# rst-tu-dortmund/teb_local_planner

Measured on AMD Instinct MI355X. Metric: TEB LM iterations/sec (whole node), higher is better.
Workload: dtype f64; 1 GPU; C4: 256 candidate TEBs/GPU x 200 poses at the start (teb_autosize on, the reference default: 193..287 poses, mean 234, after the step), 500 point obstacles (50 dynamic), diff-drive, point footprint, TebConfig defaults, 4 outer x 5 inner; tebs_per_gpu=256, tebs_total=256, poses=200, pose_capacity=288, tebs_ok=256, obstacles=500, jacobian_mode=analytic (closed form), exchange=none (single GPU), binary_hash=10be306ab42698fd, binary_variant_defines=

## Files before the change

### include/teb_amd.h

```cpp
#ifndef TEB_AMD_H_
#define TEB_AMD_H_

#include <stdint.h>

#ifdef __cplusplus
extern "C" {
#endif

#define TEB_AMD_ABI_VERSION 3
#define TEB_AMD_MAX_POSES 944

enum {
  TEB_AMD_OK = 0,
  TEB_AMD_ERR_INVALID_ARG = 1,
  TEB_AMD_ERR_NO_DEVICE = 2,
  TEB_AMD_ERR_HIP = 3,
  TEB_AMD_ERR_CAPACITY = 4,
  TEB_AMD_ERR_UNSUPPORTED = 5
};

enum {
  TEB_AMD_TEB_OK = 0,
  TEB_AMD_TEB_FAILED = 1,
  TEB_AMD_TEB_NONFINITE = 2
// ... 129 lines not shown
typedef struct teb_amd_results {
  int32_t* status;
  int32_t* lm_iterations;
  int32_t* lm_trials;
  double*  chi2;
  double*  cost;
  double*  lambda;
} teb_amd_results_t;

typedef struct teb_amd_handle teb_amd_handle_t;

int  teb_amd_abi_version(void);
const char* teb_amd_last_error(void);
void teb_amd_config_default(teb_amd_config_t* cfg);

enum { TEB_AMD_LAYOUT_AUTO = 0,
       TEB_AMD_LAYOUT_BLOCKS_LDS = 1,
       TEB_AMD_LAYOUT_BAND_LDS = 2,
       TEB_AMD_LAYOUT_BAND_HBM = 3 };
enum { TEB_AMD_HSIG3D_AUTO = 0, TEB_AMD_HSIG3D_WIDE = 1, TEB_AMD_HSIG3D_SMALL = 2 };
typedef struct teb_amd_options {
  int32_t struct_size;
  int32_t layout;
  int32_t fixed_layout;
  int32_t band_ldlt;
  int32_t generic_distance_path;
  int32_t hsig3d_kernel;
  int32_t no_near_cache;
  int32_t multi_cu;
  int32_t multi_cu_timeout_us;
  int32_t speculative_trials;
  int32_t generic_config_path;
  int32_t compile_for_config;
  int32_t reserved[4];
} teb_amd_options_t;
void teb_amd_options_default(teb_amd_options_t* opt);

int  teb_amd_create(const teb_amd_config_t* cfg, int32_t max_tebs, int32_t max_poses,
                    int32_t max_obstacles, int32_t max_obstacle_vertices, int32_t max_via_points,
                    int32_t device, void* stream, teb_amd_handle_t** out);
int  teb_amd_create_ex(const teb_amd_config_t* cfg, int32_t max_tebs, int32_t max_poses,
                       int32_t max_obstacles, int32_t max_obstacle_vertices, int32_t max_via_points,
                       int32_t device, void* stream, const teb_amd_options_t* options, teb_amd_handle_t** out);
void teb_amd_destroy(teb_amd_handle_t* h);
int  teb_amd_set_config(teb_amd_handle_t* h, const teb_amd_config_t* cfg);

int  teb_amd_set_obstacles(teb_amd_handle_t* h, const teb_amd_obstacles_t* obst);
int  teb_amd_set_via_points(teb_amd_handle_t* h, int32_t count, const double* x, const double* y);

int  teb_amd_upload_tebs(teb_amd_handle_t* h, const teb_amd_teb_batch_t* batch);
int  teb_amd_download_tebs(teb_amd_handle_t* h, teb_amd_teb_batch_t* batch);

int  teb_amd_optimize_batch(teb_amd_handle_t* h, int32_t iterations_innerloop, int32_t iterations_outerloop,
                            int32_t compute_cost_afterwards, double obst_cost_scale,
                            double viapoint_cost_scale, int32_t alternative_time_cost);
int  teb_amd_synchronize(teb_amd_handle_t* h);
int  teb_amd_get_results(teb_amd_handle_t* h, teb_amd_results_t* out);

#define TEB_AMD_ITERATION_LOG_ROWS 256
int  teb_amd_set_iteration_log(teb_amd_handle_t* h, int32_t enable);
int  teb_amd_get_iteration_log(teb_amd_handle_t* h, int32_t b, double* rows, int32_t capacity_rows, int32_t* n_rows);

int  teb_amd_select_best(teb_amd_handle_t* h, int32_t last_best, int32_t initial_plan,
                         int32_t* best, double* best_cost);

int  teb_amd_last_launch_info(teb_amd_handle_t* h, int32_t* distance_helpers_per_band, int32_t* solver_helpers_per_band,
                              int32_t* repeated_single_cu);
// ... 106 lines not shown
```

### teb_local_planner_amd/_abi.py

```python
import ctypes as C

import numpy as np

MAX_FOOTPRINT_VERTICES = 64

OK, ERR_INVALID_ARG, ERR_NO_DEVICE, ERR_HIP, ERR_CAPACITY, ERR_UNSUPPORTED = range(6)
MAX_POSES = 944
TEB_OK, TEB_FAILED, TEB_NONFINITE = range(3)
FOOTPRINT_POINT, FOOTPRINT_CIRCULAR, FOOTPRINT_TWO_CIRCLES, FOOTPRINT_LINE, FOOTPRINT_POLYGON = range(5)
OBST_POINT, OBST_CIRCULAR, OBST_LINE, OBST_PILL, OBST_POLYGON = range(5)
ROT_LEFT, ROT_NONE, ROT_RIGHT = range(3)
JACOBIAN_ANALYTIC, JACOBIAN_G2O_NUMERIC = range(2)

c_i32 = C.c_int32
c_f64 = C.c_double
p_i32 = C.POINTER(C.c_int32)
p_f64 = C.POINTER(C.c_double)


class Config(C.Structure):
    _fields_ = [
        ("teb_autosize", c_i32), ("dt_ref", c_f64), ("dt_hysteresis", c_f64),
        ("min_samples", c_i32), ("max_samples", c_i32), ("exact_arc_length", c_i32),
        ("via_points_ordered", c_i32),
# ... 36 lines not shown
        ("count", c_i32), ("type", p_i32), ("ax", p_f64), ("ay", p_f64), ("bx", p_f64), ("by", p_f64),
        ("radius", p_f64), ("vx", p_f64), ("vy", p_f64), ("dynamic", p_i32),
        ("vert_offset", p_i32), ("vert_x", p_f64), ("vert_y", p_f64),
    ]


class TebBatch(C.Structure):
    _fields_ = [
        ("count", c_i32), ("stride", c_i32), ("n", p_i32), ("x", p_f64), ("y", p_f64), ("theta", p_f64),
        ("dt", p_f64), ("has_vel_start", p_i32), ("vel_start", p_f64), ("has_vel_goal", p_i32),
        ("vel_goal", p_f64), ("prefer_rotdir", p_i32), ("via_points_enabled", p_i32),
    ]


class HcpParams(C.Structure):
    _fields_ = [
        ("simple_exploration", c_i32), ("roadmap_graph_no_samples", c_i32), ("roadmap_graph_area_width", c_f64),
        ("roadmap_graph_area_length_scale", c_f64), ("obstacle_heading_threshold", c_f64), ("xy_goal_tolerance", c_f64),
        ("max_number_classes", c_i32), ("max_number_plans_in_current_class", c_i32), ("h_signature_prescaler", c_f64),
        ("h_signature_threshold", c_f64), ("allow_init_with_backwards_motion", c_i32), ("delete_detours_backwards", c_i32),
        ("detours_orientation_tolerance", c_f64), ("length_start_orientation_vector", c_f64),
        ("max_ratio_detours_duration_best_duration", c_f64), ("global_plan_overwrite_orientation", c_i32),
        ("viapoints_all_candidates", c_i32),
    ]


LAYOUT_AUTO, LAYOUT_BLOCKS_LDS, LAYOUT_BAND_LDS, LAYOUT_BAND_HBM = 0, 1, 2, 3
HSIG3D_AUTO, HSIG3D_WIDE, HSIG3D_SMALL = 0, 1, 2


class Options(C.Structure):
    _fields_ = [("struct_size", c_i32), ("layout", c_i32), ("fixed_layout", c_i32), ("band_ldlt", c_i32),
                ("generic_distance_path", c_i32), ("hsig3d_kernel", c_i32), ("no_near_cache", c_i32), ("multi_cu", c_i32),
                ("multi_cu_timeout_us", c_i32), ("speculative_trials", c_i32), ("generic_config_path", c_i32), ("compile_for_config", c_i32), ("reserved", c_i32 * 4)]

    def __init__(self, layout=LAYOUT_AUTO, fixed_layout=False, band_ldlt=False, generic_distance_path=False, hsig3d_kernel=HSIG3D_AUTO,
                 no_near_cache=False, multi_cu=0, multi_cu_timeout_us=0, speculative_trials=0, generic_config_path=False, compile_for_config=0):
        super().__init__()
        self.struct_size = C.sizeof(Options)
        self.layout = {"auto": LAYOUT_AUTO, "cr": LAYOUT_BLOCKS_LDS, "band": LAYOUT_BAND_LDS, "bandg": LAYOUT_BAND_HBM}.get(layout, layout)
        self.fixed_layout = int(fixed_layout)
        self.band_ldlt = int(band_ldlt)
        self.generic_distance_path = int(generic_distance_path)
        self.hsig3d_kernel = {"auto": HSIG3D_AUTO, "wide": HSIG3D_WIDE, "small": HSIG3D_SMALL}.get(hsig3d_kernel, hsig3d_kernel)
        self.no_near_cache = int(no_near_cache)
        self.multi_cu = int(multi_cu)
        self.multi_cu_timeout_us = int(multi_cu_timeout_us)
        self.speculative_trials = int(speculative_trials)
        self.generic_config_path = int(generic_config_path)
        self.compile_for_config = int(compile_for_config)


class Results(C.Structure):
    _fields_ = [
        ("status", p_i32), ("lm_iterations", p_i32), ("lm_trials", p_i32), ("chi2", p_f64),
        ("cost", p_f64), ("lambda_", p_f64),
    ]


def _ptr(a, ty):
    if a is None:
        return C.cast(None, C.POINTER(ty))
    return a.ctypes.data_as(C.POINTER(ty))


def f64(a):
    return np.ascontiguousarray(a, dtype=np.float64)


def i32(a):
    return np.ascontiguousarray(a, dtype=np.int32)


class ObstacleTable:

    def __init__(self):
        self.type, self.ax, self.ay, self.bx, self.by = [], [], [], [], []
        self.radius, self.vx, self.vy, self.dynamic = [], [], [], []
        self.vert_offset, self.vert_x, self.vert_y = [0], [], []
        self._frozen = None

    def _add(self, ty, ax=0.0, ay=0.0, bx=0.0, by=0.0, r=0.0, verts=None, vel=None):
        self._frozen = None
# ... 173 lines not shown
```

### teb_local_planner_amd/csrc/teb_amd.hip

```cpp
#include <hip/hip_runtime.h>

#include <chrono>
#include <cmath>
#include <cstdio>
#include <unistd.h>
#include <cstdlib>
#include <algorithm>
#include <cstring>
#include <limits>
#include <string>
#include <random>
#include <vector>

#include "../../include/teb_amd.h"
#include "../../include/teb_amd_debug.h"
#define TEB_AMD_MAIN_TU
#include "teb_kernel.hpp"
#include "teb_opt_launch.hpp"
#include "teb_fleet.hpp"
#include "teb_strip.hpp"
#include "teb_hsig.hpp"
#include "teb_graph.hpp"
#include "teb_comm.hpp"
#include "teb_rtc.hpp"
// ... 1293 lines not shown
  const size_t w = (size_t)(bt->stride < h->stride ? bt->stride : h->stride) * sizeof(double);
  const size_t hp = (size_t)bt->stride * sizeof(double), dp = (size_t)h->stride * sizeof(double);
  HIPCHK(hipMemcpy2DAsync(bt->x, hp, h->x.p, dp, w, B, hipMemcpyDeviceToHost, h->stream));
  HIPCHK(hipMemcpy2DAsync(bt->y, hp, h->y.p, dp, w, B, hipMemcpyDeviceToHost, h->stream));
  HIPCHK(hipMemcpy2DAsync(bt->theta, hp, h->th.p, dp, w, B, hipMemcpyDeviceToHost, h->stream));
  HIPCHK(hipMemcpy2DAsync(bt->dt, hp, h->dt.p, dp, w, B, hipMemcpyDeviceToHost, h->stream));
  HIPCHK(hipStreamSynchronize(h->stream));
  for (int b = 0; b < B; ++b) bt->n[b] = n[b];
  return TEB_AMD_OK;
}

int teb_amd_optimize_batch(teb_amd_handle_t* h, int32_t inner, int32_t outer, int32_t compute_cost, double obst_cost_scale,
                           double viapoint_cost_scale, int32_t alternative_time_cost) {
  int rc = check_handle(h);
  if (rc) return rc;
  if (inner < 0 || outer < 0) return fail(TEB_AMD_ERR_INVALID_ARG, "negative iteration count");
  const bool fleet = h->fleet.n_scenes > 0;
  if (fleet) {
#ifndef TEB_AMD_HAS_FLEET_UNITS
    return fail(TEB_AMD_ERR_UNSUPPORTED, "fleet launches exist in the product library only; this one is the variant built with [" TEB_AMD_VARIANT_DEFINES "]");
#else
    if (h->cfg.jacobian_mode != TEB_AMD_JACOBIAN_ANALYTIC)
      return fail(TEB_AMD_ERR_INVALID_ARG, "fleet launches need jacobian_mode TEB_AMD_JACOBIAN_ANALYTIC");
    for (int b = 0; b < h->B; ++b)
      if (h->fleet.band_scene[b] >= h->fleet.n_scenes) {
        char buf[160];
        std::snprintf(buf, sizeof buf, "band %d maps to scene %d, but %d scenes are set (teb_amd_set_band_scenes)", b, h->fleet.band_scene[b], h->fleet.n_scenes);
        return fail(TEB_AMD_ERR_INVALID_ARG, buf);
      }
#endif
  }
  OptArgs a;
  std::memset(&a, 0, sizeof a);
  a.inner = inner; a.outer = outer; a.compute_cost = compute_cost; a.no_near_cache = h->opt.no_near_cache != 0; a.band_ldlt = (fleet ? h->fleet.solver : h->solver) == SOLVER_BANDG ? 0 : h->band_ldlt; a.Hband = h->Hband.p; a.hband_stride = h->hband_stride;
  a.obst_scale = obst_cost_scale; a.via_scale = viapoint_cost_scale; a.alt_time = alternative_time_cost;
  if (h->iter_log_on) { a.iter_log = h->iter_log.p; a.iter_log_cap = TEB_AMD_ITERATION_LOG_ROWS; }
  if (h->phase_log_on) a.phase_log = h->phase_log.p;
#ifdef TEB_PROFILE
  a.dbg_H = h->dbg_H.p;
#endif
  h->last_inner = inner;
  return launch(h, a);
}

int teb_amd_set_iteration_log(teb_amd_handle_t* h, int32_t enable) {
  int rc = check_handle(h);
  if (rc) return rc;
  if (enable && !h->iter_log.p) {
    const size_t count = (size_t)h->max_tebs * TEB_AMD_ITERATION_LOG_ROWS * 4;
    HIPCHK(h->iter_log.alloc(count));
    HIPCHK(hipMemsetAsync(h->iter_log.p, 0, count * sizeof(double), h->stream));
  }
  h->iter_log_on = enable != 0;
  return TEB_AMD_OK;
}

static_assert(kPhaseLogSlots == TEB_AMD_PHASE_LOG_SLOTS, "teb_amd_debug.h and teb_device.hpp disagree");
int teb_amd_set_phase_log(teb_amd_handle_t* h, int32_t enable) {
  int rc = check_handle(h);
  if (rc) return rc;
  if (enable && !h->phase_log.p) {
    const size_t count = (size_t)h->max_tebs * kPhaseLogSlots;
    HIPCHK(h->phase_log.alloc(count));
    HIPCHK(hipMemsetAsync(h->phase_log.p, 0, count * sizeof(double), h->stream));
  }
  h->phase_log_on = enable != 0;
  return TEB_AMD_OK;
// ... 1696 lines not shown
```

### teb_local_planner_amd/csrc/teb_device.hpp

```cpp
#pragma once
#include <hip/hip_runtime.h>
#include <stdint.h>

#include "../../include/teb_amd.h"

#define TEB_PF_ALL(X)                                                                                                              \
  X(EXACT_ARC) X(COST_EXPONENT) X(NEW_ASSOCIATION) X(DYNAMIC_EDGES) X(VIA_POINTS) X(NONHOLONOMIC_VELOCITY) X(VELOCITY_EDGES)      \
  X(ACCELERATION_EDGES) X(NONHOLONOMIC_ACCELERATION) X(TIME_OPTIMAL) X(SHORTEST_PATH) X(VELOCITY_OBSTACLE_RATIO) X(RADIUS_FREE)   \
  X(DEBUG_LINEARIZE) X(BAND_LDLT) X(INFLATED) X(NO_NEAR_CACHE) X(DIVERGENCE_DETECTION) X(KIN_DIFF_DRIVE) X(KIN_EDGES)
#define TEB_PF_EXPR_EXACT_ARC (c.exact_arc_length)
#define TEB_PF_DFLT_EXACT_ARC false
#define TEB_PF_EXPR_COST_EXPONENT (c.obstacle_cost_exponent != 1.0 && c.min_obstacle_dist > 0.0)
#define TEB_PF_DFLT_COST_EXPONENT false
#define TEB_PF_EXPR_NEW_ASSOCIATION (!c.legacy_obstacle_association)
#define TEB_PF_DFLT_NEW_ASSOCIATION true
#define TEB_PF_EXPR_DYNAMIC_EDGES (c.include_dynamic_obstacles && c.weight_obstacle != 0)
#define TEB_PF_DFLT_DYNAMIC_EDGES true
#define TEB_PF_HOST_DYNAMIC_EDGES (c.weight_obstacle != 0)
#define TEB_PF_EXPR_VIA_POINTS (sc.nvia > 0 && c.weight_viapoint != 0)
#define TEB_PF_DFLT_VIA_POINTS false
#define TEB_PF_WIDE_VIA_POINTS 1
#define TEB_PF_EXPR_NONHOLONOMIC_VELOCITY (c.max_vel_y == 0)
#define TEB_PF_DFLT_NONHOLONOMIC_VELOCITY true
#define TEB_PF_WIDE_NONHOLONOMIC_VELOCITY 1
// ... 187 lines not shown
  const double* vs;
  const int* has_vg;
  const double* vg;
  const int* rotdir;
  const int* via_en;
  int* status;
  int* optimized;
  int* iters;
  int* last_iters;
  int* trials;
  double* chi2;
  double* cost;
  double* lambda;
  int* assoc_cnt;
  int* assoc;
  int assoc_cap;
  int* assoc_overflow;
  int* legacy_idx;
  int* via_pose;
  int via_cap;
  double* Hbackup;
  size_t hmat_stride;
  long long* clk;
};

struct OptArgs {
  int inner, outer, compute_cost;
  double obst_scale, via_scale;
  int alt_time;
  double* Hband;
  size_t hband_stride;
  int band_ldlt;
  int no_near_cache;
  double* iter_log;
  int iter_log_cap;
  int debug_linearize;
  double debug_weight_multiplier;
  double* dbg_H;
  double* dbg_b;
  double* dbg_chi2;
  double* phase_log;
};
constexpr int kPhaseLogSlots = 9;

}
```

### teb_local_planner_amd/csrc/teb_kernel.hpp

```cpp
#pragma once
#include "teb_edges.hpp"
#include "teb_multicu.hpp"
#include "teb_autoresize_chain.hpp"

namespace tebamd {

#ifdef TEB_PROFILE
#define PROF_DECL long long prof_t0 = 0, prof_wg_t0 = clock64(), prof_acc[8] = {0, 0, 0, 0, 0, 0, 0, 0};
#define PROF_START() prof_t0 = clock64()
#define PROF_END(k) prof_acc[k] += clock64() - prof_t0
#else
#define PROF_DECL const bool plog_ = args.phase_log != nullptr; long long* const plog_acc_ = reinterpret_cast<long long*>(l.red + 40); \
  if (plog_ && threadIdx.x == 0) { for (int q_ = 0; q_ < 9; ++q_) plog_acc_[q_] = 0; plog_acc_[9] = clock64(); }
#define PROF_START() do { if (plog_ && threadIdx.x == 0) plog_acc_[8] = clock64(); } while (0)
#define PROF_END(k) do { if (plog_ && threadIdx.x == 0) plog_acc_[k] += clock64() - plog_acc_[8]; } while (0)
#endif

#ifdef TEB_PROFILE
__device__ long long g_ev_prof[8];
#define EVP_DECL long long evp_t0 = clock64(), evp_t1;
#define EVP(k) do { __builtin_amdgcn_sched_barrier(0); asm volatile("s_waitcnt vmcnt(0) lgkmcnt(0)" ::: "memory"); evp_t1 = clock64(); __builtin_amdgcn_sched_barrier(0); if (blockIdx.x == 0 && threadIdx.x == 1) g_ev_prof[k] += evp_t1 - evp_t0; evp_t0 = evp_t1; } while (0)
__device__ unsigned long long g_assoc_stats[4];
__device__ unsigned long long g_ar_steps[4];
__device__ unsigned long long g_near_recomputed, g_near_queries;
__device__ long long g_lin_prof[16];
#define LNP_DECL long long lnp_t0 = clock64(), lnp_t1;
#define LNP(k) do { __builtin_amdgcn_sched_barrier(0); asm volatile("s_waitcnt vmcnt(0) lgkmcnt(0)" ::: "memory"); lnp_t1 = clock64(); __builtin_amdgcn_sched_barrier(0); if (blockIdx.x == 0 && threadIdx.x == 0) g_lin_prof[k] += lnp_t1 - lnp_t0; lnp_t0 = lnp_t1; } while (0)
#elif defined(TEB_AMD_STAMP)
#define EVP_DECL long long evp_t0 = clock64();
#define EVP(k) do { const long long t_ = clock64(); if ((k) == (TEB_AMD_STAMP) && threadIdx.x == 1) reinterpret_cast<long long*>(l.red + 40)[7] += t_ - evp_t0; evp_t0 = t_; } while (0)
#define LNP_DECL long long lnp_t0 = clock64();
#define LNP(k) do { const long long t_ = clock64(); if ((k) + 10 == (TEB_AMD_STAMP) && threadIdx.x == 0) reinterpret_cast<long long*>(l.red + 40)[7] += t_ - lnp_t0; lnp_t0 = t_; } while (0)
#else
#define EVP_DECL
#define EVP(k)
#define LNP_DECL
#define LNP(k)
#endif
#ifdef TEB_AMD_POINTS_KEEP_GENERIC
#define TEB_IF_FAST(F) if ((F) && sc.fast_points)
#define TEB_IF_NOT_FAST(F) if (!((F) && sc.fast_points))
#else
#define TEB_IF_FAST(F) if constexpr (F)
#define TEB_IF_NOT_FAST(F) if constexpr (!(F))
#endif
enum { SOLVER_BAND = 0, SOLVER_CR = 1, SOLVER_BANDG = 2 };
typedef double teb_v2d __attribute__((ext_vector_type(2)));
constexpr int kBlk = 66;
// ... 538 lines not shown
    const int G = (k0 > 0 || kThreads > 256) ? lanes_per_pose(n - 1 - k0) : 1;
    const int i = k0 + tid / G, sl = tid % G;
    const bool active = i <= n - 2;
    constexpr int EM = JMODE == TEB_AMD_JACOBIAN_G2O_NUMERIC ? 2 : 1;
    const unsigned long long near = active ? dyn_near_cached<EM, FAST>(c, sc, l, i, sl, G, nc, pass) : 0ull;
    LNP(2);
    A.clear();
    if (active) eval_index<EM, FAST>(c, sc, t, l, i, A, near, sl, G);
    LNP(3);
    if (G > 1) {
      for (int off = 1; off < G; off <<= 1) {
#pragma unroll
        for (int q = 0; q < 6; ++q) A.H[q] += __shfl_xor(A.H[q], off, 64);
#pragma unroll
        for (int q = 0; q < 3; ++q) A.g[q] += __shfl_xor(A.g[q], off, 64);
      }
    }
    LNP(4);
    if (active && sl == 0) scatter<SOLVER, 0>(A, l, i, n);
    __syncthreads();
    if (active && sl == 0) scatter<SOLVER, 1>(A, l, i, n);
    __syncthreads();
    if (active && sl == 0) scatter<SOLVER, 2>(A, l, i, n);
    __syncthreads();
    LNP(5);
    k0 += kThreads / G;
  }
  if (tid < 3) { *diag_ptr<SOLVER>(l, tid) = 1.0; l.bv[tid] = 0; }
  if (tid >= 4 && tid < 8) { int r = 4 * (n - 1) + (tid - 4); *diag_ptr<SOLVER>(l, r) = 1.0; l.bv[r] = 0; }
  if (SOLVER == SOLVER_CR && tid >= 8 && tid < 12 && (n & 1)) {
    int r = 4 * n + (tid - 8); *diag_ptr<SOLVER>(l, r) = 1.0;
  }
  cats[0] = A.chi[0]; cats[1] = A.chi[1]; cats[2] = A.chi[2]; cats[3] = A.chi[3];
  block_sum<4>(cats, l.red);
  LNP(6);
}

template <bool FAST, int PART>
__device__ __forceinline__ void evaluate_pass(const teb_amd_config_t& c, const SceneDev& sc, const TebCtx& t, const Lds& l, NearCache& nc, Accum& A) {
  for (int k0 = 0, pass = 0; k0 < t.n - 1; ++pass) {
    const int G = (k0 > 0 || kThreads > 256) ? lanes_per_pose(t.n - 1 - k0) : 1;
    const int i = k0 + (int)threadIdx.x / G;
    if (i <= t.n - 2) {
      const unsigned long long near = dyn_near_cached<0, FAST>(c, sc, l, i, (int)threadIdx.x % G, G, nc, pass);
      eval_index<0, FAST, PART>(c, sc, t, l, i, A, near, (int)threadIdx.x % G, G);
    }
    k0 += kThreads / G;
  }
}
template <bool FAST>
__device__ inline void evaluate(const teb_amd_config_t& c, const SceneDev& sc, const TebCtx& t, const Lds& l, NearCache& nc,
                                double* cats , bool trig_is_current = false) {
  if (!trig_is_current) {
    refresh_trig(l, t.n);
    __syncthreads();
  }
  Accum A;
  A.clear_chi();
  evaluate_pass<FAST, 0>(c, sc, t, l, nc, A);
  cats[0] = A.chi[0]; cats[1] = A.chi[1]; cats[2] = A.chi[2]; cats[3] = A.chi[3];
  block_sum<5>(cats, l.red);
}
__device__ inline bool evaluate_mcu(const teb_amd_config_t& c, const SceneDev& sc, const TebCtx& t, const Lds& l, NearCache& nc, McuMaster& m, int S,
                                    double* cats ) {
  refresh_trig(l, t.n);
  __syncthreads();
  mcu_publish(m, l.sx, l.sy, l.cs, l.sn, l.tdyn, t.n, S);
// ... 1808 lines not shown
        __builtin_amdgcn_s_sleep(2);
      }
      l.ired[24] = (int)cmd;
      l.ired[25] = (int)ld_agent_u32(ctl + MCU_SN);
      if (cmd != kMcuSpecExit) __builtin_amdgcn_fence(__ATOMIC_ACQUIRE, "agent");
    }
    __syncthreads();
    const unsigned cmd = (unsigned)l.ired[24];
    const int n = l.ired[25];
    __syncthreads();
    if (cmd == kMcuSpecExit || n < 2 || n > plan.S) return;
    __builtin_amdgcn_fence(__ATOMIC_ACQUIRE, "agent");
    epoch = cmd;
    mcu_trace(mc.trace, epoch, 0x61);
    const int Nt = 4 * n;
    const double lambda = in[4 * S + 8 + k];
    for (int r = tid; r < Nt + 8; r += kThreads) l.bv[r] = r < Nt ? in[r] : 0.0;
    if constexpr (SOLVER == SOLVER_CR) {
      const int hsz = ((Nt + 7) >> 3) * 2 * kBlk;
      hmat_load<SOLVER_CR>(l, hsz, Nt, Hbk);
    }
    __syncthreads();
    if constexpr (SOLVER == SOLVER_CR) cr_solve_blocks_helper(plan, sc, n, lambda);
    else cr_solve_hybrid_helper(plan, n, lambda, Hbk);
    for (int r = tid; r < Nt; r += kThreads) st_agent_f64(out + r, l.dxv[r]);
    if (tid == 0) st_agent_f64(out + 4 * S + 8, l.ired[0] != 0 ? 1.0 : 0.0);
    asm volatile("s_waitcnt vmcnt(0)" ::: "memory");
    __syncthreads();
    if (tid == 0) st_agent_u32(ctl + MCU_SDONE + k, epoch);
    mcu_trace(mc.trace, epoch, 0x62);
  }
}

enum { SCENE_POINTS = 0, SCENE_GENERIC = 1, SCENE_POINTS_SMALL = 2, SCENE_GENERIC_SMALL = 3, SCENE_POINTS_DEFAULTS = 4, SCENE_POINTS_SMALL_DEFAULTS = 5,
       SCENE_GENERIC_DEFAULTS = 6, SCENE_GENERIC_SMALL_DEFAULTS = 7, SCENE_POINTS_WIDE = 8, SCENE_POINTS_SMALL_WIDE = 9,
       SCENE_POINTS_LIGHT = 10, SCENE_POINTS_SMALL_LIGHT = 11,
       SCENE_POINTS_CUSTOM = 12, SCENE_POINTS_SMALL_CUSTOM = 13, SCENE_GENERIC_CUSTOM = 14, SCENE_GENERIC_SMALL_CUSTOM = 15 };
template <int SOLVER, int JMODE, int SCENE>
__global__ void __launch_bounds__(kThreads)
#ifdef TEB_AMD_FLEET
teb_optimize_kernel(const teb_amd_config_t c, const FleetDev fl, const BatchDev bt, const OptArgs args,
                    const LdsPlan plan, const McuDev mc) {
#else
teb_optimize_kernel(const teb_amd_config_t c, const SceneDev sc, const BatchDev bt, const OptArgs args,
                    const LdsPlan plan, const McuDev mc) {
#endif
  extern __shared__ __attribute__((aligned(16))) double lds_base[];
  constexpr bool FAST = SCENE == SCENE_POINTS || SCENE == SCENE_POINTS_SMALL || SCENE == SCENE_POINTS_DEFAULTS || SCENE == SCENE_POINTS_SMALL_DEFAULTS ||
                        SCENE == SCENE_POINTS_WIDE || SCENE == SCENE_POINTS_SMALL_WIDE || SCENE == SCENE_POINTS_LIGHT || SCENE == SCENE_POINTS_SMALL_LIGHT ||
                        SCENE == SCENE_POINTS_CUSTOM || SCENE == SCENE_POINTS_SMALL_CUSTOM;
  constexpr bool MCU = SCENE == SCENE_POINTS_SMALL || SCENE == SCENE_GENERIC_SMALL || SCENE == SCENE_POINTS_SMALL_DEFAULTS ||
                       SCENE == SCENE_GENERIC_SMALL_DEFAULTS || SCENE == SCENE_POINTS_SMALL_WIDE || SCENE == SCENE_POINTS_SMALL_LIGHT ||
                       SCENE == SCENE_POINTS_SMALL_CUSTOM || SCENE == SCENE_GENERIC_SMALL_CUSTOM;
#ifdef TEB_AMD_DEFAULTS_PROFILE
  static_assert(SCENE >= SCENE_POINTS_DEFAULTS, "a unit compiled with the profile holds a *_DEFAULTS kind");
#else
  static_assert(SCENE < SCENE_POINTS_DEFAULTS, "*_DEFAULTS kinds need -DTEB_AMD_DEFAULTS_PROFILE");
#endif
#ifdef TEB_AMD_PROFILE_ANY_KINEMATICS
  static_assert(SCENE == SCENE_GENERIC_DEFAULTS || SCENE == SCENE_GENERIC_SMALL_DEFAULTS, "the generic-shape kinds of the profile keep the kinematics flags");
#endif
#ifdef TEB_AMD_PROFILE_CUSTOM
  static_assert(SCENE >= SCENE_POINTS_CUSTOM, "-DTEB_AMD_PROFILE_CUSTOM builds the *_CUSTOM kinds");
#else
  static_assert(SCENE < SCENE_POINTS_CUSTOM, "*_CUSTOM kinds are compiled at run time (teb_rtc.hpp)");
#endif
// ... 161 lines not shown
            double ddx = vx - l.sx[i], ddy = vy - l.sy[i];
            double d2 = ddx * ddx + ddy * ddy;
            if (d2 < best) { best = d2; bi = i; }
          }
          index = block_argmin(best, bi, l.red, l.ired);
          if (index == 0x7fffffff) index = -1;
        }
        if (c.via_points_ordered) start_pose_idx = index + 2;
        if (index > n - 2) index = n - 2;
        int attach = index;
        if (index < 1) attach = c.via_points_ordered ? 1 : -1;
        if (tid == 0) via_pose[v] = attach;
      }
    } else {
      for (int v = tid; v < sc.nvia; v += kThreads) via_pose[v] = -1;
    }
    __threadfence_block();
    __syncthreads();
    LNP(11);
    PROF_END(1);

    near_cache.invalidate();
    if (args.inner <= 0 && !TEB_CFGI(DEBUG_LINEARIZE)) { status = TEB_AMD_TEB_FAILED; break; }
    t.mcu.items = nullptr;
    if (mcu_on && obst_edges && !(mc.debug_flags & 2)) {
      mcu_publish(mm, l.sx, l.sy, l.cs, l.sn, l.tdyn, n, S);
      mcu_issue(mm, MCU_KIND_DIST, n);
      if (!mcu_wait(mm, l.ired + 26)) { status = TEB_AMD_TEB_FAILED; if (tid == 0) or_agent_i32(bt.assoc_overflow + b, 4); break; }
      t.mcu.items = mcu_items;
    }
    double ni = 2;
    bool lm_ok = true;
    last_iters = 0;
    for (int it = 0; it < args.inner && lm_ok; ++it) {
      double cats[4];
      PROF_START();
      linearize<SOLVER, JMODE, FAST>(c, sc, t, l, near_cache, cats, !trig_stale);
      trig_stale = false;
      PROF_END(2);
      double currentChi = ((cats[0] + cats[1]) + cats[2]) + cats[3];
      if (TEB_CFGI(DEBUG_LINEARIZE)) {
        if (b == 0) {
          const int Nt = 4 * n;
          for (int q = tid; q < Nt * kBand; q += kThreads) {
            const int r = q / kBand, d = q % kBand, cc = r - d;
            double v = 0;
            if (cc >= 0) {
              if (SOLVER != SOLVER_CR) v = l.Hb[hbo(r) + d];
              else if ((r >> 3) == (cc >> 3)) v = l.Db[(r >> 3) * kBlk + (r & 7) * 8 + (cc & 7)];
              else if ((r >> 3) == (cc >> 3) + 1) v = l.Lb[(r >> 3) * kBlk + (r & 7) * 8 + (cc & 7)];
            }
            args.dbg_H[q] = v;
          }
          for (int q = tid; q < Nt; q += kThreads) args.dbg_b[q] = l.bv[q];
          if (tid < 4) args.dbg_chi2[tid] = cats[tid];
        }
        done = true;
        break;
      }
      const int Nt = 4 * n;
      if (it == 0) {
        double m = 0;
        for (int r = tid; r < Nt; r += kThreads)
          if (r >= 3 && r < 4 * (n - 1)) m = fmax(m, fabs(*diag_ptr<SOLVER>(l, r)));
        lambda = 1e-5 * block_max(m, l.red);
        ni = 2;
      }
      PROF_START();
      const int hsz = (SOLVER != SOLVER_CR) ? hbo(Nt) : ((Nt + 7) >> 3) * 2 * kBlk;
      const bool keep_copy = !(SOLVER != SOLVER_CR && !TEB_CFGI(BAND_LDLT));
      if constexpr (MCU) {
        if (spec_on) spec_wait_idle(mm, l.ired + 26);
      }
      const bool spec_now = MCU && spec_on && !mm.spec_failed;
#ifndef TEB_AMD_DIAG_EDGE_ONLY
      if (keep_copy) {
        if (spec_now) {
          for (int q = tid; q < hsz; q += kThreads) st_agent_f64(Hbk + q, *hmat_ptr<SOLVER>(l, q, Nt));
        } else {
          hmat_save<SOLVER>(l, hsz, Nt, Hbk);
        }
      }
      if (SOLVER == SOLVER_BAND && !TEB_CFGI(BAND_LDLT)) cr_copy_band(l, n, Hbk, spec_now);
#endif
      if constexpr (MCU) {
        if (spec_now) spec_issue(mm, l.bv, Nt, n, S, lambda, ni);
      }
      PROF_END(3);
      double rho = 0;
      int qmax = 0;
      bool h_spent = false;
      do {
        PROF_START();
        bool taken = false;
        if constexpr (MCU) {
          if (spec_now && !mm.spec_failed && qmax >= 1 && qmax <= mm.K)
            taken = spec_take(mm, qmax, l.dxv, l.ired, Nt, S, l.ired + 26);
        }
#ifdef TEB_AMD_DIAG_EDGE_ONLY
        taken = true;
        for (int r = tid; r < Nt; r += kThreads) l.dxv[r] = (r >= 3 && r < 4 * (n - 1)) ? l.bv[r] / (*diag_ptr<SOLVER>(l, r) + lambda) : 0.0;
        if (tid == 0) l.ired[0] = 1;
        __syncthreads();
#endif
        if (!taken) {
        if (keep_copy && h_spent) {
          hmat_load<SOLVER>(l, hsz, Nt, Hbk);
          __syncthreads();
        }
        h_spent = true;
        if constexpr (SOLVER == SOLVER_BAND) {
          if (TEB_CFGI(BAND_LDLT)) {
            if (tid < 64) {
              bool ok = banded_ldlt_solve_wave0(l, Nt, lambda);
              if (tid == 0) l.ired[0] = ok ? 1 : 0;
            }
            __syncthreads();
          } else {
            cr_solve_hybrid(plan, n, lambda, Hbk);
          }
        } else if constexpr (SOLVER == SOLVER_BANDG) {
          cr_solve_t<true, true>(plan, sc, n, lambda, Hbk, l.Hb);
        } else {
          cr_solve_t<false, false>(plan, sc, n, lambda, nullptr, nullptr);
        }
        }
        PROF_END(4);
        PROF_START();
        const bool ok2 = l.ired[0] != 0;
        if (!ok2) { for (int r = tid; r < Nt; r += kThreads) l.dxv[r] = l.bv[r]; __syncthreads(); }
        double bx_[kMaxPoseIter], by_[kMaxPoseIter], bth_[kMaxPoseIter], bdt_[kMaxPoseIter];
        double sc_part = 0;
#pragma unroll
        for (int kk = 0; kk < kMaxPoseIter; ++kk) {
          const int i = tid + kk * kThreads;
          if (i < n) {
            bx_[kk] = l.sx[i]; by_[kk] = l.sy[i]; bth_[kk] = l.sth[i]; bdt_[kk] = l.sdt[i];
            if (i >= 1 && i <= n - 2) {
              l.sx[i] += l.dxv[4 * i]; l.sy[i] += l.dxv[4 * i + 1];
              const double th_new = normalize_theta(l.sth[i] + l.dxv[4 * i + 2]);
              l.sth[i] = th_new;
              double sv, cv;
              sincos(th_new, &sv, &cv);
              l.cs[i] = cv; l.sn[i] = sv;
            }
            if (i <= n - 2) l.sdt[i] += l.dxv[4 * i + 3];
#pragma unroll
            for (int q = 0; q < 4; ++q) {
              double xj = l.dxv[4 * i + q];
              sc_part += xj * (lambda * xj + l.bv[4 * i + q]);
            }
          }
        }
        __syncthreads();
        trig_stale = false;
        double tc[5];
        tc[4] = sc_part;
        if (MCU && t.mcu.items != nullptr) {
          if (!evaluate_mcu(c, sc, t, l, near_cache, mm, S, tc)) { status = TEB_AMD_TEB_FAILED; if (tid == 0) or_agent_i32(bt.assoc_overflow + b, 4); done = true; lm_ok = false; break; }
        } else
          evaluate<FAST>(c, sc, t, l, near_cache, tc, true);
        last_cats[0] = tc[0]; last_cats[1] = tc[1]; last_cats[2] = tc[2]; last_cats[3] = tc[3];
        double tempChi = ((tc[0] + tc[1]) + tc[2]) + tc[3];
        double scv[1] = {tc[4]};
        PROF_END(5);
        PROF_START();
        if (!ok2) tempChi = 1.7976931348623157e308;
        rho = (currentChi - tempChi);
        double scale = scv[0] + 1e-3;
        rho /= scale;
        ++trials;
        if (rho > 0 && isfinite(tempChi)) {
          double alpha = 1. - pow((2 * rho - 1), 3);
          alpha = fmin(alpha, 2. / 3.);
          double scaleFactor = fmax(1. / 3., alpha);
          lambda *= scaleFactor;
          ni = 2;
          currentChi = tempChi;
        } else {
          lambda *= ni;
          ni *= 2;
#pragma unroll
          for (int kk = 0; kk < kMaxPoseIter; ++kk) {
            const int i = tid + kk * kThreads;
            if (i < n) { l.sx[i] = bx_[kk]; l.sy[i] = by_[kk]; l.sth[i] = bth_[kk]; l.sdt[i] = bdt_[kk]; }
          }
          trig_stale = true;
          if (!isfinite(lambda)) { ++qmax; __syncthreads(); break; }
        }
        __syncthreads();
        PROF_END(6);
        qmax++;
      } while (rho < 0 && qmax < 10);
      if (args.iter_log && tid == 0 && iters < args.iter_log_cap) {
        double* row = args.iter_log + ((size_t)b * args.iter_log_cap + iters) * 4;
        row[0] = currentChi; row[1] = lambda; row[2] = (double)qmax; row[3] = (double)n;
      }
      ++iters;
      ++last_iters;
      chi2_final = currentChi;
      if (qmax == 10 || rho == 0 || !isfinite(lambda)) lm_ok = false;
      if (TEB_CFGI(DIVERGENCE_DETECTION)) {
        double fc[5];
        fc[4] = 0;
        if (MCU && t.mcu.items != nullptr) {
          if (!evaluate_mcu(c, sc, t, l, near_cache, mm, S, fc)) { status = TEB_AMD_TEB_FAILED; if (tid == 0) or_agent_i32(bt.assoc_overflow + b, 4); done = true; break; }
        } else
          evaluate<FAST>(c, sc, t, l, near_cache, fc, !trig_stale);
          trig_stale = false;
        last_cats[0] = fc[0]; last_cats[1] = fc[1]; last_cats[2] = fc[2]; last_cats[3] = fc[3];
        chi2_final = ((fc[0] + fc[1]) + fc[2]) + fc[3];
      }
    }
    if (done) break;
    if (args.compute_cost && outer == args.outer - 1) {
      double cst = 0;
      if (args.alt_time) {
        double s[1] = {0};
        for (int i = tid; i < n - 1; i += kThreads) s[0] += l.sdt[i];
        block_sum<1>(s, l.red);
        cst += s[0];
      }
      cst += last_cats[CAT_OBST] * args.obst_scale;
      cst += last_cats[CAT_VIA] * args.via_scale;
      if (!args.alt_time) cst += last_cats[CAT_TIME];
      cst += last_cats[CAT_OTHER];
// ... 40 lines not shown
```

### teb_local_planner_amd/planner.py

```python
import ctypes as C
import os

import numpy as np

from . import _abi
from .config import TebConfig

_HERE = os.path.dirname(os.path.abspath(__file__))
_LIB = None


class TebAmdError(RuntimeError):
    def __init__(self, code, what, msg):
        super().__init__("%s failed: status %d (%s)" % (what, code, msg))
        self.code = code


def lib():
    global _LIB
    if _LIB is None:
        so = os.environ.get("TEB_AMD_LIB") or os.path.join(_HERE, "libteb_amd.so")
        if not os.path.exists(so):
            raise TebAmdError(-1, "load", "libteb_amd.so missing: run `python -m teb_local_planner_amd.build`")
        L = C.CDLL(so)
# ... 178 lines not shown
    def optimize(self, inner, outer, compute_cost=False, obst_cost_scale=1.0, viapoint_cost_scale=1.0,
                 alternative_time_cost=False):
        _chk(lib().teb_amd_optimize_batch(self._h, inner, outer, int(compute_cost), float(obst_cost_scale),
                                          float(viapoint_cost_scale), int(alternative_time_cost)),
             "teb_amd_optimize_batch")

    def synchronize(self):
        _chk(lib().teb_amd_synchronize(self._h), "teb_amd_synchronize")

    def results(self):
        res = _abi.ResultsHost(self.count)
        rs = res.c_struct()
        _chk(lib().teb_amd_get_results(self._h, C.byref(rs)), "teb_amd_get_results")
        return res

    def set_iteration_log(self, enable=True):
        _chk(lib().teb_amd_set_iteration_log(self._h, int(bool(enable))), "teb_amd_set_iteration_log")

    PHASES = ("autoresize", "graph side data", "linearize", "H backup", "solve", "update + evaluate", "accept / restore")

    def set_phase_log(self, enable=True):
        L = lib()
        L.teb_amd_set_phase_log.argtypes = [C.c_void_p, C.c_int32]
        _chk(L.teb_amd_set_phase_log(self._h, int(bool(enable))), "teb_amd_set_phase_log")

    def phase_log(self):
        L = lib()
        L.teb_amd_get_phase_log.argtypes = [C.c_void_p, _abi.p_f64, C.c_int32, _abi.p_i32]
        self._sync_count()
        out = np.zeros((max(self.count, 1), 9)); nb = C.c_int32(0)
        _chk(L.teb_amd_get_phase_log(self._h, _abi._ptr(out, C.c_double), self.count, C.byref(nb)), "teb_amd_get_phase_log")
        return out[:nb.value]

    def iteration_log(self, b, capacity_rows=256):
        rows = np.zeros((int(capacity_rows), 4))
        n = C.c_int32(0)
        _chk(lib().teb_amd_get_iteration_log(self._h, int(b), _abi._ptr(rows, C.c_double), int(capacity_rows), C.byref(n)),
             "teb_amd_get_iteration_log")
        return rows[:n.value].copy()

    def select_best(self, last_best=-1, initial_plan=-1):
        best = C.c_int32(-1)
        cost = C.c_double(0)
        _chk(lib().teb_amd_select_best(self._h, last_best, initial_plan, C.byref(best), C.byref(cost)),
             "teb_amd_select_best")
        return best.value, cost.value

    def select_best_distributed(self, comm, global_offset, last_best_global=-1, initial_plan_global=-1):
        best = C.c_int32(-1); cost = C.c_double(0); owner = C.c_int32(-1)
        _chk(lib().teb_amd_select_best_distributed(self._h, comm._c, int(global_offset), int(last_best_global), int(initial_plan_global),
                                                   C.byref(best), C.byref(cost), C.byref(owner)), "teb_amd_select_best_distributed")
        return best.value, cost.value, owner.value

    def broadcast_band(self, comm, owner_rank, local_index, capacity=None):
        cap = int(capacity or self.max_poses)
        n = C.c_int32(0)
        x = np.zeros(cap); y = np.zeros(cap); th = np.zeros(cap); dt = np.zeros(cap)
        P = lambda a: _abi._ptr(a, C.c_double)
        _chk(lib().teb_amd_broadcast_band(self._h, comm._c, int(owner_rank), int(local_index), cap, C.byref(n), P(x), P(y), P(th), P(dt)),
             "teb_amd_broadcast_band")
        return x[:n.value].copy(), y[:n.value].copy(), th[:n.value].copy(), dt[:max(n.value - 1, 0)].copy()

    def last_kernel_ms(self):
        ms = C.c_float(0)
        _chk(lib().teb_amd_last_kernel_ms(self._h, C.byref(ms)), "teb_amd_last_kernel_ms")
        return ms.value
# ... 672 lines not shown
```

Before: 2.551 million TEB.LM-iterations/s.

## Speculatively linearize at trial point instead of separate evaluate when acceptance expected

Restructures the LM inner loop so that, when a heuristic predicts the trial step will be accepted, the kernel runs a full linearize at the trial state in place of the plain cost evaluation. On acceptance the already-built system is reused for the next iteration, which saves one evaluate pass per accepted step. On rejection the extra Jacobian/Hessian assembly is wasted work. The change also widens a block reduction to five values, adds an option to disable the speculation, and packs counters into the phase log.

```diff
diff --git a/include/teb_amd.h b/include/teb_amd.h
--- a/include/teb_amd.h
+++ b/include/teb_amd.h
@@ -185,7 +185,8 @@
   int32_t speculative_trials;
   int32_t generic_config_path;
   int32_t compile_for_config;
-  int32_t reserved[4];
+  int32_t no_speculative_linearize;
+  int32_t reserved[3];
 } teb_amd_options_t;
 void teb_amd_options_default(teb_amd_options_t* opt);
 
diff --git a/teb_local_planner_amd/_abi.py b/teb_local_planner_amd/_abi.py
--- a/teb_local_planner_amd/_abi.py
+++ b/teb_local_planner_amd/_abi.py
@@ -92,10 +92,12 @@
 class Options(C.Structure):
     _fields_ = [("struct_size", c_i32), ("layout", c_i32), ("fixed_layout", c_i32), ("band_ldlt", c_i32),
                 ("generic_distance_path", c_i32), ("hsig3d_kernel", c_i32), ("no_near_cache", c_i32), ("multi_cu", c_i32),
-                ("multi_cu_timeout_us", c_i32), ("speculative_trials", c_i32), ("generic_config_path", c_i32), ("compile_for_config", c_i32), ("reserved", c_i32 * 4)]
+                ("multi_cu_timeout_us", c_i32), ("speculative_trials", c_i32), ("generic_config_path", c_i32), ("compile_for_config", c_i32), ("no_speculative_linearize", c_i32),
+                ("reserved", c_i32 * 3)]
 
     def __init__(self, layout=LAYOUT_AUTO, fixed_layout=False, band_ldlt=False, generic_distance_path=False, hsig3d_kernel=HSIG3D_AUTO,
-                 no_near_cache=False, multi_cu=0, multi_cu_timeout_us=0, speculative_trials=0, generic_config_path=False, compile_for_config=0):
+                 no_near_cache=False, multi_cu=0, multi_cu_timeout_us=0, speculative_trials=0, generic_config_path=False, compile_for_config=0,
+                 no_speculative_linearize=False):
         super().__init__()
         self.struct_size = C.sizeof(Options)
         self.layout = {"auto": LAYOUT_AUTO, "cr": LAYOUT_BLOCKS_LDS, "band": LAYOUT_BAND_LDS, "bandg": LAYOUT_BAND_HBM}.get(layout, layout)
@@ -109,6 +111,7 @@
         self.speculative_trials = int(speculative_trials)
         self.generic_config_path = int(generic_config_path)
         self.compile_for_config = int(compile_for_config)
+        self.no_speculative_linearize = int(no_speculative_linearize)
 
 
 class Results(C.Structure):
diff --git a/teb_local_planner_amd/csrc/teb_amd.hip b/teb_local_planner_amd/csrc/teb_amd.hip
--- a/teb_local_planner_amd/csrc/teb_amd.hip
+++ b/teb_local_planner_amd/csrc/teb_amd.hip
@@ -1349,7 +1349,7 @@
   }
   OptArgs a;
   std::memset(&a, 0, sizeof a);
-  a.inner = inner; a.outer = outer; a.compute_cost = compute_cost; a.no_near_cache = h->opt.no_near_cache != 0; a.band_ldlt = (fleet ? h->fleet.solver : h->solver) == SOLVER_BANDG ? 0 : h->band_ldlt; a.Hband = h->Hband.p; a.hband_stride = h->hband_stride;
+  a.inner = inner; a.outer = outer; a.compute_cost = compute_cost; a.no_near_cache = h->opt.no_near_cache != 0; a.no_speculative_linearize = h->opt.no_speculative_linearize != 0; a.band_ldlt = (fleet ? h->fleet.solver : h->solver) == SOLVER_BANDG ? 0 : h->band_ldlt; a.Hband = h->Hband.p; a.hband_stride = h->hband_stride;
   a.obst_scale = obst_cost_scale; a.via_scale = viapoint_cost_scale; a.alt_time = alternative_time_cost;
   if (h->iter_log_on) { a.iter_log = h->iter_log.p; a.iter_log_cap = TEB_AMD_ITERATION_LOG_ROWS; }
   if (h->phase_log_on) a.phase_log = h->phase_log.p;
diff --git a/teb_local_planner_amd/csrc/teb_device.hpp b/teb_local_planner_amd/csrc/teb_device.hpp
--- a/teb_local_planner_amd/csrc/teb_device.hpp
+++ b/teb_local_planner_amd/csrc/teb_device.hpp
@@ -243,6 +243,7 @@
   size_t hband_stride;
   int band_ldlt;
   int no_near_cache;
+  int no_speculative_linearize;
   double* iter_log;
   int iter_log_cap;
   int debug_linearize;
diff --git a/teb_local_planner_amd/csrc/teb_kernel.hpp b/teb_local_planner_amd/csrc/teb_kernel.hpp
--- a/teb_local_planner_amd/csrc/teb_kernel.hpp
+++ b/teb_local_planner_amd/csrc/teb_kernel.hpp
@@ -14,6 +14,11 @@
   if (plog_ && threadIdx.x == 0) { for (int q_ = 0; q_ < 9; ++q_) plog_acc_[q_] = 0; plog_acc_[9] = clock64(); }
 #define PROF_START() do { if (plog_ && threadIdx.x == 0) plog_acc_[8] = clock64(); } while (0)
 #define PROF_END(k) do { if (plog_ && threadIdx.x == 0) plog_acc_[k] += clock64() - plog_acc_[8]; } while (0)
+#endif
+#if !defined(TEB_PROFILE) && !defined(TEB_AMD_STAMP)
+#define LIN_AHEAD_COUNT(v) do { if (plog_ && threadIdx.x == 0) plog_acc_[7] += (v); } while (0)
+#else
+#define LIN_AHEAD_COUNT(v) do { } while (0)
 #endif
 
 #ifdef TEB_PROFILE
@@ -618,7 +623,7 @@
     int r = 4 * n + (tid - 8); *diag_ptr<SOLVER>(l, r) = 1.0;
   }
   cats[0] = A.chi[0]; cats[1] = A.chi[1]; cats[2] = A.chi[2]; cats[3] = A.chi[3];
-  block_sum<4>(cats, l.red);
+  block_sum<5>(cats, l.red);
   LNP(6);
 }
 
@@ -2493,6 +2498,11 @@
   }
 }
 
+__device__ __forceinline__ bool lm_expect_accept(int it, int q, int prev_trials, double last_scale) {
+  if (it == 0) return q >= 4;
+  return q >= 1 || prev_trials >= 3 || (it <= 2 && last_scale <= 1. / 3.);
+}
+
 enum { SCENE_POINTS = 0, SCENE_GENERIC = 1, SCENE_POINTS_SMALL = 2, SCENE_GENERIC_SMALL = 3, SCENE_POINTS_DEFAULTS = 4, SCENE_POINTS_SMALL_DEFAULTS = 5,
        SCENE_GENERIC_DEFAULTS = 6, SCENE_GENERIC_SMALL_DEFAULTS = 7, SCENE_POINTS_WIDE = 8, SCENE_POINTS_SMALL_WIDE = 9,
        SCENE_POINTS_LIGHT = 10, SCENE_POINTS_SMALL_LIGHT = 11,
@@ -2720,65 +2730,27 @@
     double ni = 2;
     bool lm_ok = true;
     last_iters = 0;
+    const bool lin_ahead_on = SOLVER != SOLVER_BANDG && JMODE == TEB_AMD_JACOBIAN_ANALYTIC && !args.no_speculative_linearize &&
+                              !TEB_CFGI(DEBUG_LINEARIZE) && !TEB_CFGI(DIVERGENCE_DETECTION);
+    bool sys_ready = false;
+    int prev_trials = 0;
+    double last_scale = 1.0;
+    double currentChi = 0;
     for (int it = 0; it < args.inner && lm_ok; ++it) {
-      double cats[4];
-      PROF_START();
-      linearize<SOLVER, JMODE, FAST>(c, sc, t, l, near_cache, cats, !trig_stale);
-      trig_stale = false;
-      PROF_END(2);
-      double currentChi = ((cats[0] + cats[1]) + cats[2]) + cats[3];
-      if (TEB_CFGI(DEBUG_LINEARIZE)) {
-        if (b == 0) {
-          const int Nt = 4 * n;
-          for (int q = tid; q < Nt * kBand; q += kThreads) {
-            const int r = q / kBand, d = q % kBand, cc = r - d;
-            double v = 0;
-            if (cc >= 0) {
-              if (SOLVER != SOLVER_CR) v = l.Hb[hbo(r) + d];
-              else if ((r >> 3) == (cc >> 3)) v = l.Db[(r >> 3) * kBlk + (r & 7) * 8 + (cc & 7)];
-              else if ((r >> 3) == (cc >> 3) + 1) v = l.Lb[(r >> 3) * kBlk + (r & 7) * 8 + (cc & 7)];
-            }
-            args.dbg_H[q] = v;
-          }
-          for (int q = tid; q < Nt; q += kThreads) args.dbg_b[q] = l.bv[q];
-          if (tid < 4) args.dbg_chi2[tid] = cats[tid];
-        }
-        done = true;
-        break;
-      }
       const int Nt = 4 * n;
-      if (it == 0) {
-        double m = 0;
-        for (int r = tid; r < Nt; r += kThreads)
-          if (r >= 3 && r < 4 * (n - 1)) m = fmax(m, fabs(*diag_ptr<SOLVER>(l, r)));
-        lambda = 1e-5 * block_max(m, l.red);
-        ni = 2;
-      }
-      PROF_START();
       const int hsz = (SOLVER != SOLVER_CR) ? hbo(Nt) : ((Nt + 7) >> 3) * 2 * kBlk;
       const bool keep_copy = !(SOLVER != SOLVER_CR && !TEB_CFGI(BAND_LDLT));
-      if constexpr (MCU) {
-        if (spec_on) spec_wait_idle(mm, l.ired + 26);
-      }
-      const bool spec_now = MCU && spec_on && !mm.spec_failed;
-#ifndef TEB_AMD_DIAG_EDGE_ONLY
-      if (keep_copy) {
-        if (spec_now) {
-          for (int q = tid; q < hsz; q += kThreads) st_agent_f64(Hbk + q, *hmat_ptr<SOLVER>(l, q, Nt));
-        } else {
-          hmat_save<SOLVER>(l, hsz, Nt, Hbk);
-        }
-      }
-      if (SOLVER == SOLVER_BAND && !TEB_CFGI(BAND_LDLT)) cr_copy_band(l, n, Hbk, spec_now);
-#endif
-      if constexpr (MCU) {
-        if (spec_now) spec_issue(mm, l.bv, Nt, n, S, lambda, ni);
-      }
-      PROF_END(3);
+      bool spec_now = false;
       double rho = 0;
       int qmax = 0;
       bool h_spent = false;
-      do {
+      bool open = true;
+      for (;;) {
+        double tc[5];
+        tc[4] = 0;
+        bool ok2 = true, ahead = false;
+        double bx_[kMaxPoseIter], by_[kMaxPoseIter], bth_[kMaxPoseIter], bdt_[kMaxPoseIter];
+        if (!open) {
         PROF_START();
         bool taken = false;
         if constexpr (MCU) {
@@ -2815,9 +2787,8 @@
         }
         PROF_END(4);
         PROF_START();
-        const bool ok2 = l.ired[0] != 0;
+        ok2 = l.ired[0] != 0;
         if (!ok2) { for (int r = tid; r < Nt; r += kThreads) l.dxv[r] = l.bv[r]; __syncthreads(); }
-        double bx_[kMaxPoseIter], by_[kMaxPoseIter], bth_[kMaxPoseIter], bdt_[kMaxPoseIter];
         double sc_part = 0;
 #pragma unroll
         for (int kk = 0; kk < kMaxPoseIter; ++kk) {
@@ -2842,12 +2813,80 @@
         }
         __syncthreads();
         trig_stale = false;
-        double tc[5];
         tc[4] = sc_part;
-        if (MCU && t.mcu.items != nullptr) {
-          if (!evaluate_mcu(c, sc, t, l, near_cache, mm, S, tc)) { status = TEB_AMD_TEB_FAILED; if (tid == 0) or_agent_i32(bt.assoc_overflow + b, 4); done = true; lm_ok = false; break; }
-        } else
-          evaluate<FAST>(c, sc, t, l, near_cache, tc, true);
+        ahead = lin_ahead_on && ok2 && it + 1 < args.inner && !(MCU && (t.mcu.items != nullptr || spec_now)) &&
+                lm_expect_accept(it, qmax, prev_trials, last_scale);
+        }
+        if (open ? !sys_ready : ahead) {
+          if (!open) PROF_END(5);
+          PROF_START();
+          Lds lt = l;
+          if (!open) lt.bv = l.dxv;
+          linearize<SOLVER, JMODE, FAST>(c, sc, t, lt, near_cache, tc, !trig_stale);
+          trig_stale = false;
+          PROF_END(2);
+          PROF_START();
+        } else if (!open) {
+          if (MCU && t.mcu.items != nullptr) {
+            if (!evaluate_mcu(c, sc, t, l, near_cache, mm, S, tc)) { status = TEB_AMD_TEB_FAILED; if (tid == 0) or_agent_i32(bt.assoc_overflow + b, 4); done = true; lm_ok = false; break; }
+          } else
+            evaluate<FAST>(c, sc, t, l, near_cache, tc, true);
+        }
+        if (open) {
+          if (sys_ready) {
+            for (int q = 2 * tid; q < Nt + 8; q += 2 * kThreads) *reinterpret_cast<teb_v2d*>(l.bv + q) = *reinterpret_cast<const teb_v2d*>(l.dxv + q);
+            __syncthreads();
+            sys_ready = false;
+          } else {
+            currentChi = ((tc[0] + tc[1]) + tc[2]) + tc[3];
+          }
+          if (TEB_CFGI(DEBUG_LINEARIZE)) {
+            if (b == 0) {
+              for (int q = tid; q < Nt * kBand; q += kThreads) {
+                const int r = q / kBand, d = q % kBand, cc = r - d;
+                double v = 0;
+                if (cc >= 0) {
+                  if (SOLVER != SOLVER_CR) v = l.Hb[hbo(r) + d];
+                  else if ((r >> 3) == (cc >> 3)) v = l.Db[(r >> 3) * kBlk + (r & 7) * 8 + (cc & 7)];
+                  else if ((r >> 3) == (cc >> 3) + 1) v = l.Lb[(r >> 3) * kBlk + (r & 7) * 8 + (cc & 7)];
+                }
+                args.dbg_H[q] = v;
+              }
+              for (int q = tid; q < Nt; q += kThreads) args.dbg_b[q] = l.bv[q];
+              if (tid < 4) args.dbg_chi2[tid] = tc[tid];
+            }
+            done = true;
+            break;
+          }
+          if (it == 0) {
+            double m = 0;
+            for (int r = tid; r < Nt; r += kThreads)
+              if (r >= 3 && r < 4 * (n - 1)) m = fmax(m, fabs(*diag_ptr<SOLVER>(l, r)));
+            lambda = 1e-5 * block_max(m, l.red);
+            ni = 2;
+          }
+          PROF_START();
+          if constexpr (MCU) {
+            if (spec_on) spec_wait_idle(mm, l.ired + 26);
+          }
+          spec_now = MCU && spec_on && !mm.spec_failed;
+#ifndef TEB_AMD_DIAG_EDGE_ONLY
+          if (keep_copy) {
+            if (spec_now) {
+              for (int q = tid; q < hsz; q += kThreads) st_agent_f64(Hbk + q, *hmat_ptr<SOLVER>(l, q, Nt));
+            } else {
+              hmat_save<SOLVER>(l, hsz, Nt, Hbk);
+            }
+          }
+          if (SOLVER == SOLVER_BAND && !TEB_CFGI(BAND_LDLT)) cr_copy_band(l, n, Hbk, spec_now);
+#endif
+          if constexpr (MCU) {
+            if (spec_now) spec_issue(mm, l.bv, Nt, n, S, lambda, ni);
+          }
+          PROF_END(3);
+          open = false;
+          continue;
+        }
         last_cats[0] = tc[0]; last_cats[1] = tc[1]; last_cats[2] = tc[2]; last_cats[3] = tc[3];
         double tempChi = ((tc[0] + tc[1]) + tc[2]) + tc[3];
         double scv[1] = {tc[4]};
@@ -2865,6 +2904,9 @@
           lambda *= scaleFactor;
           ni = 2;
           currentChi = tempChi;
+          last_scale = scaleFactor;
+          sys_ready = ahead;
+          if (ahead) LIN_AHEAD_COUNT(1LL + (1LL << 20));
         } else {
           lambda *= ni;
           ni *= 2;
@@ -2874,12 +2916,16 @@
             if (i < n) { l.sx[i] = bx_[kk]; l.sy[i] = by_[kk]; l.sth[i] = bth_[kk]; l.sdt[i] = bdt_[kk]; }
           }
           trig_stale = true;
+          if (ahead) LIN_AHEAD_COUNT(1LL + (1LL << 40));
           if (!isfinite(lambda)) { ++qmax; __syncthreads(); break; }
         }
         __syncthreads();
         PROF_END(6);
         qmax++;
-      } while (rho < 0 && qmax < 10);
+        if (!(rho < 0 && qmax < 10)) break;
+      }
+      if (TEB_CFGI(DEBUG_LINEARIZE)) break;
+      prev_trials = qmax;
       if (args.iter_log && tid == 0 && iters < args.iter_log_cap) {
         double* row = args.iter_log + ((size_t)b * args.iter_log_cap + iters) * 4;
         row[0] = currentChi; row[1] = lambda; row[2] = (double)qmax; row[3] = (double)n;
diff --git a/teb_local_planner_amd/planner.py b/teb_local_planner_amd/planner.py
--- a/teb_local_planner_amd/planner.py
+++ b/teb_local_planner_amd/planner.py
@@ -234,6 +234,10 @@
         _chk(L.teb_amd_get_phase_log(self._h, _abi._ptr(out, C.c_double), self.count, C.byref(nb)), "teb_amd_get_phase_log")
         return out[:nb.value]
 
+    def speculation_counters(self):
+        packed = self.phase_log()[:, 7].astype(np.int64)
+        return np.stack([packed & 0xFFFFF, (packed >> 20) & 0xFFFFF, packed >> 40], axis=1)
+
     def iteration_log(self, b, capacity_rows=256):
         rows = np.zeros((int(capacity_rows), 4))
         n = C.c_int32(0)
```

Result: no change. 2.531 million TEB.LM-iterations/s (-0.8%).
